# kezakool/flair-for-aigle

Hardware: AMD Instinct MI355X
Metric: 512x512x5 tiles/sec (train fwd+bwd+AdamW), U-Net ResNet-34, 19 classes (higher is better)
Workload: dtype bf16; 1 GPU; synthetic 512x512x5 tiles, 19-class U-Net (ResNet-34 encoder), batch 32 per GPU, train step (BASELINE.json configs[1]); global_batch=32, tile=512, parallelism=dp1

## Files before the change

### flair-for-aigle_amd/csrc/conv_pack.hip

```cpp
#include "ffa_common.h"

#include "conv7x7_stem.h"

struct PackDesc {
  const float* src;
  void* dst;
  const float* scale;
  long long s_row, s_ch;
  int rows, chs;
  int flip, kh, kw;
  int nchunks;
  int rg, bco, ncb;
  int ncb64;
  int mt, ci;
};


__device__ __forceinline__ void pack_eight(const PackDesc& p, long long i8, int dtype) {
  const int EPC = (dtype == FFA_BF16) ? 16 : 8;
  const int G8 = EPC / 8;
  const int taps = p.rg * p.kw;
  const int nrg = p.kh / p.rg;
  long long t = i8;
  const int e0 = (int)(t % G8) * 8; t /= G8;
  const int tap = t % taps; t /= taps;
  const int row_l = t % p.bco; t /= p.bco;
  const int rg = t % nrg; t /= nrg;
  const int cc = t % p.nchunks; t /= p.nchunks;
  const int cb = (int)t;
  int row_in_block = row_l;
  if (p.bco >= 64) {
    const int j = row_l & 63, mt = j >> 5, rho = j & 31;
    row_in_block = (row_l & ~63) + 16 * (rho >> 3) + 8 * ((rho >> 2) & 1) + 4 * mt + (rho & 3);
  }
  const int row = cb * p.bco + row_in_block;
  const int ch0 = cc * EPC + e0;
  int r = rg * p.rg + tap / p.kw;
  int sx = tap % p.kw;
  if (p.flip) {
    r = p.kh - 1 - r;
    sx = p.kw - 1 - sx;
  }
  float v[8];
  const bool row_ok = row < p.rows;
  const float sc = (row_ok && p.scale) ? p.scale[row] : 1.f;
  const float* src = p.src + (long long)row * p.s_row + r * p.kw + sx;
#pragma unroll
  for (int j = 0; j < 8; ++j) {
    const int ch = ch0 + j;
    v[j] = (row_ok && ch < p.chs) ? src[(long long)ch * p.s_ch] * sc : 0.f;
  }
  if (dtype == FFA_BF16)
    ffa_store8<ffa_bf16>(static_cast<ffa_bf16*>(p.dst) + i8 * 8, v);
  else
    ffa_store8<float>(static_cast<float*>(p.dst) + i8 * 8, v);
}

__global__ void pack_igemm_kernel(PackDesc one, const PackDesc* __restrict__ table, int dtype) {
  PackDesc p = one;
  if (table) p = table[blockIdx.y];
  const int EPC = (dtype == FFA_BF16) ? 16 : 8;
  const long long total8 = (long long)p.ncb * p.nchunks * (p.kh / p.rg) * p.bco * (p.rg * p.kw) * (EPC / 8);
  for (long long i = blockIdx.x * (long long)blockDim.x + threadIdx.x; i < total8;
       i += (long long)gridDim.x * blockDim.x)
    pack_eight(p, i, dtype);
}


template <typename T>
__device__ __forceinline__ void ring_pack_piece(const PackDesc& p, long long i16) {
  constexpr int EPF = ElemTraits<T>::kPerFrag;
  long long t = i16;
  const int hp = (int)(t % 2); t /= 2;
  const int row_l = (int)(t % 64); t /= 64;
  const int ks = (int)(t % 2); t /= 2;
  const int s = (int)(t % 3); t /= 3;
  const int r = (int)(t % 3); t /= 3;
  const int cc = (int)(t % p.nchunks); t /= p.nchunks;
  const int cb = (int)t;
  const int mt = row_l >> 5, rho = row_l & 31;
  const int row = cb * 64 + 16 * (rho >> 3) + 8 * ((rho >> 2) & 1) + 4 * mt + (rho & 3);
  const int hsrc = hp ^ ((row_l >> 3) & 1);
  const int ch0 = cc * (4 * EPF) + ks * (2 * EPF) + hsrc * EPF;
  int rr = r, ss = s;
  if (p.flip) {
    rr = 2 - r;
    ss = 2 - s;
  }
  float v[8];
  const bool row_ok = row < p.rows;
  const float sc = (row_ok && p.scale) ? p.scale[row] : 1.f;
  const float* src = p.src + (long long)row * p.s_row + rr * 3 + ss;
#pragma unroll
  for (int j = 0; j < EPF; ++j) {
    const int ch = ch0 + j;
    v[j] = (row_ok && ch < p.chs) ? src[(long long)ch * p.s_ch] * sc : 0.f;
  }
  if constexpr (EPF == 8) {
    ffa_store8<ffa_bf16>(static_cast<ffa_bf16*>(p.dst) + i16 * 8, v);
  } else {
    *reinterpret_cast<float4*>(static_cast<float*>(p.dst) + i16 * 4) = make_float4(v[0], v[1], v[2], v[3]);
  }
}

__device__ __forceinline__ void ring16_pack_rowslot(const PackDesc& p, long long idx) {
  long long t = idx;
  int row_l, sp, cc;
  if (!p.flip) {
    sp = (int)(t % 4); t /= 4;
    cc = (int)(t % p.nchunks); t /= p.nchunks;
    row_l = (int)(t % 64); t /= 64;
  } else {
    row_l = (int)(t % 64); t /= 64;
    sp = (int)(t % 4); t /= 4;
    cc = (int)(t % p.nchunks); t /= p.nchunks;
  }
  const int cb = (int)t;
  const int mt = row_l >> 4, kg = (row_l >> 2) & 3, i = row_l & 3;
  const int row = cb * 64 + 16 * kg + 4 * mt + i;
  const int slot = sp ^ (((row_l >> 2) & 1) << 1);
  const int ch0 = cc * 32 + slot * 8;
  const bool row_ok = row < p.rows;
  const float sc = (row_ok && p.scale) ? p.scale[row] : 1.f;
  float v[8][9];
  if (!p.flip && row_ok && ch0 + 8 <= p.chs && (p.s_row & 3) == 0 && ((size_t)p.src & 15) == 0) {
    const ffa_f32x4* src4 = reinterpret_cast<const ffa_f32x4*>(p.src + (long long)row * p.s_row + (long long)ch0 * 9);
    float f[72];
#pragma unroll
    for (int q = 0; q < 18; ++q) {
      const ffa_f32x4 t4 = src4[q];
      f[4 * q] = t4[0]; f[4 * q + 1] = t4[1]; f[4 * q + 2] = t4[2]; f[4 * q + 3] = t4[3];
    }
#pragma unroll
    for (int j = 0; j < 8; ++j)
#pragma unroll
      for (int tp = 0; tp < 9; ++tp) v[j][tp] = f[j * 9 + tp] * sc;
  } else {
#pragma unroll
    for (int j = 0; j < 8; ++j) {
      const int ch = ch0 + j;
      const bool ok = row_ok && ch < p.chs;
      const float* src = p.src + (long long)(ok ? row : 0) * p.s_row + (long long)(ok ? ch : 0) * p.s_ch;
#pragma unroll
      for (int tp = 0; tp < 9; ++tp) v[j][tp] = ok ? src[p.flip ? 8 - tp : tp] * sc : 0.f;
    }
  }
  ffa_bf16* dst = static_cast<ffa_bf16*>(p.dst) + ((((long long)cb * p.nchunks + cc) * 9) * 256 + row_l * 4 + sp) * 8;
#pragma unroll
  for (int tp = 0; tp < 9; ++tp) {
    float o[8];
#pragma unroll
    for (int j = 0; j < 8; ++j) o[j] = v[j][tp];
    ffa_store8<ffa_bf16>(dst + (long long)tp * 256 * 8, o);
  }
}

__global__ void pack_ring_kernel(PackDesc one, const PackDesc* __restrict__ table, int dtype) {
  PackDesc p = one;
  if (table) p = table[blockIdx.y];
  if (dtype == FFA_BF16) {
    const long long total = (long long)p.ncb64 * p.nchunks * 64 * 4;
    for (long long i = blockIdx.x * (long long)blockDim.x + threadIdx.x; i < total; i += (long long)gridDim.x * blockDim.x)
      ring16_pack_rowslot(p, i);
    return;
  }
  const long long total = (long long)p.ncb64 * p.nchunks * 3 * 3 * 2 * 64 * 2;
  for (long long i = blockIdx.x * (long long)blockDim.x + threadIdx.x; i < total; i += (long long)gridDim.x * blockDim.x)
    ring_pack_piece<float>(p, i);
}


__device__ __forceinline__ void thin_pack_piece(const PackDesc& p, int idx) {
  const int ks_n = (p.ci == 32) ? 9 : 5;
  const int lane = idx % 64;
  const int ks = (idx / 64) % ks_n;
  const int mt = idx / (64 * ks_n);
  const int r = lane & 15, kg = lane >> 4;
  const int q = r >> 2, i = r & 3;
  const int row = (p.mt == 2) ? (8 * q + 4 * mt + i) : (4 * q + i);
  int tap, ch0;
  if (p.ci == 32) {
    tap = ks;
    ch0 = 8 * kg;
  } else {
    tap = 2 * ks + (kg >> 1);
    ch0 = 8 * (kg & 1);
  }
  float v[8];
  const bool ok = row < p.rows && tap < 9;
  const float sc = (ok && p.scale) ? p.scale[row] : 1.f;
  const int st = p.flip ? 8 - tap : tap;
#pragma unroll
  for (int j = 0; j < 8; ++j) {
    const int ch = ch0 + j;
    v[j] = (ok && ch < p.chs) ? p.src[(long long)row * p.s_row + (long long)ch * p.s_ch + st] * sc : 0.f;
  }
  ffa_store8<ffa_bf16>(static_cast<ffa_bf16*>(p.dst) + (long long)idx * 8, v);
}

__global__ void pack_thin_kernel(PackDesc one, const PackDesc* __restrict__ table) {
  PackDesc p = one;
  if (table) p = table[blockIdx.y];
  const int total = p.mt * ((p.ci == 32) ? 9 : 5) * 64;
  for (int i = blockIdx.x * blockDim.x + threadIdx.x; i < total; i += gridDim.x * blockDim.x) thin_pack_piece(p, i);
}


__global__ void pack_stem_kernel(PackDesc one, const PackDesc* __restrict__ table) {
  PackDesc p = one;
  if (table) p = table[blockIdx.y];
  const int i = blockIdx.x * blockDim.x + threadIdx.x;
  if (i >= StemGeom::KSTEPS * 64 * 4) return;
  const int slotp = i & 3, rho = (i >> 2) & 63, ks = i >> 8;
  const int slot = slotp ^ (((rho >> 2) & 1) << 1);
  const int r = ks >> 1, s = 4 * (ks & 1) + slot;
  const int mt = rho >> 4, q = (rho >> 2) & 3, ii = rho & 3;
  const int co = 16 * q + 4 * mt + ii;
  unsigned short v[8];
#pragma unroll
  for (int c = 0; c < 8; ++c) {
    float x = 0.f;
    if (co < p.rows && c < p.chs && s < 7) {
      x = p.src[((size_t)(co * p.chs + c) * 7 + r) * 7 + s];
      if (p.scale) x *= p.scale[co];
    }
    v[c] = ffa_f32_to_bf16_bits(x);
  }
  uint4 u;
  u.x = v[0] | ((unsigned)v[1] << 16);
  u.y = v[2] | ((unsigned)v[3] << 16);
  u.z = v[4] | ((unsigned)v[5] << 16);
  u.w = v[6] | ((unsigned)v[7] << 16);
  reinterpret_cast<uint4*>(p.dst)[i] = u;
}


static int pack_fill(PackDesc& p, const float* w_oihw, const float* scale, void* dst, int O, int I_total, int col0,
                     int ncols, int kh, int kw, int transpose, int co_rows, int ci_pitch, int bco, int rg, int dtype) {
  FFA_REQUIRE(dtype == FFA_BF16 || dtype == FFA_F32, "pack: bad dtype");
  FFA_REQUIRE(w_oihw && dst, "pack: null pointer");
  FFA_REQUIRE(col0 >= 0 && ncols > 0 && col0 + ncols <= I_total, "pack: column block outside the tensor");
  const int eb = (dtype == FFA_BF16) ? 2 : 4;
  memset(&p, 0, sizeof(p));
  p.src = w_oihw + (long long)col0 * kh * kw;
  p.dst = dst;
  p.scale = scale;
  if (!transpose) {
    p.rows = O; p.chs = ncols;
    p.s_row = (long long)I_total * kh * kw;
    p.s_ch = (long long)kh * kw;
    p.flip = 0;
  } else {
    p.rows = ncols; p.chs = O;
    p.s_row = (long long)kh * kw;
    p.s_ch = (long long)I_total * kh * kw;
    p.flip = 1;
  }
  p.kh = kh; p.kw = kw;
  FFA_REQUIRE(p.rows <= co_rows && p.chs <= ci_pitch, "pack: padded dims smaller than the tensor");
  FFA_REQUIRE(ncols == I_total || !(bco & (FFA_BCO_STEM | FFA_BCO_THIN | FFA_BCO_RING)),
              "pack: a column block needs the conv_igemm layout");
  if (bco & FFA_BCO_STEM) {
    FFA_REQUIRE(kh == 7 && kw == 7 && dtype == FFA_BF16 && !transpose, "pack: the stem layout is for the bf16 7x7 forward operand");
    FFA_REQUIRE(O > 0 && O <= 64 && ncols > 0 && ncols <= 8, "stem pack: 1..64 output and 1..8 input channels, got %d / %d", O, ncols);
  } else if (bco & FFA_BCO_THIN) {
    FFA_REQUIRE(kh == 3 && kw == 3 && dtype == FFA_BF16, "pack: the thin layout is for bf16 3x3 kernels");
    FFA_REQUIRE((co_rows == 16 || co_rows == 32) && (ci_pitch == 16 || ci_pitch == 32), "thin pack: rows %d / pitch %d",
                co_rows, ci_pitch);
    p.mt = co_rows / 16;
    p.ci = ci_pitch;
  } else if (bco & FFA_BCO_RING) {
    FFA_REQUIRE(kh == 3 && kw == 3, "pack: the ring layout is for 3x3 kernels");
    FFA_REQUIRE(co_rows % 64 == 0 && (ci_pitch * eb) % 64 == 0, "ring pack: rows %d / pitch %d not whole groups", co_rows,
                ci_pitch);
    p.nchunks = ci_pitch * eb / 64;
    p.ncb64 = co_rows / 64;
  } else {
    FFA_REQUIRE(bco > 0 && co_rows % bco == 0, "pack: rows %d not a multiple of block %d", co_rows, bco);
    FFA_REQUIRE(rg > 0 && kh % rg == 0, "pack: bad row group");
    FFA_REQUIRE(ci_pitch % 16 == 0, "pack: channel pitch must be a multiple of 16");
    p.rg = rg; p.bco = bco;
    p.nchunks = ci_pitch * eb / 32;
    p.ncb = co_rows / bco;
  }
  return FFA_OK;
}

static int pack_launch(int dtype, int bco, const PackDesc& one, const PackDesc* table, int n, hipStream_t stream) {
  if (bco & FFA_BCO_STEM) {
    hipLaunchKernelGGL(pack_stem_kernel, dim3(ffa_cdiv(StemGeom::KSTEPS * 64 * 4, 256), n), dim3(256), 0, stream, one, table);
    return ffa_check_launch("pack_stem");
  }
  if (bco & FFA_BCO_THIN) {
    hipLaunchKernelGGL(pack_thin_kernel, dim3(5, n), dim3(256), 0, stream, one, table);
    return ffa_check_launch("pack_thin");
  }
  if (bco & FFA_BCO_RING) {
    hipLaunchKernelGGL(pack_ring_kernel, dim3(256, n), dim3(256), 0, stream, one, table, dtype);
    return ffa_check_launch("pack_ring");
  }
  hipLaunchKernelGGL(pack_igemm_kernel, dim3(256, n), dim3(256), 0, stream, one, table, dtype);
  return ffa_check_launch("pack_igemm");
}

extern "C" long long ffa_pack_conv_weight_bytes(int dtype, int co_rows, int ci_pitch, int kh, int kw, int bco) {
  if (bco & FFA_BCO_STEM) return StemGeom::WBYTES;
  if (bco & FFA_BCO_THIN) return (long long)(co_rows / 16) * ((ci_pitch == 32) ? 9 : 5) * 1024;
  const long long eb = (dtype == FFA_BF16) ? 2 : 4;
  return (long long)co_rows * ci_pitch * kh * kw * eb;
}

extern "C" int ffa_pack_conv_weight(int dtype, const float* w_oihw, const float* scale, void* dst, int O, int I,
                                    int kh, int kw, int transpose, int co_rows, int ci_pitch, int bco, int rg,
                                    hipStream_t stream) {
  PackDesc p;
  const int rc = pack_fill(p, w_oihw, scale, dst, O, I, 0, I, kh, kw, transpose, co_rows, ci_pitch, bco, rg, dtype);
  if (rc != FFA_OK) return rc;
  return pack_launch(dtype, bco, p, nullptr, 1, stream);
}

extern "C" int ffa_pack_desc_bytes(void) { return (int)sizeof(PackDesc); }

extern "C" int ffa_pack_desc_fill(void* host_desc, const float* w_oihw, const float* scale, void* dst, int O,
                                  int I_total, int col0, int ncols, int kh, int kw, int transpose, int co_rows,
                                  int ci_pitch, int bco, int rg, int dtype) {
  FFA_REQUIRE(host_desc, "pack_desc_fill: null pointer");
  PackDesc p;
  const int rc = pack_fill(p, w_oihw, scale, dst, O, I_total, col0, ncols, kh, kw, transpose, co_rows, ci_pitch, bco, rg,
                           dtype);
  if (rc != FFA_OK) return rc;
  memcpy(host_desc, &p, sizeof(p));
  return FFA_OK;
}

extern "C" int ffa_pack_conv_weights_batched(int dtype, int bco, const void* descs_device, int n, hipStream_t stream) {
  FFA_REQUIRE(dtype == FFA_BF16 || dtype == FFA_F32, "pack_batched: bad dtype");
  FFA_REQUIRE(descs_device && n > 0 && n <= 65535, "pack_batched: bad descriptor table");
  return pack_launch(dtype, bco, PackDesc{}, static_cast<const PackDesc*>(descs_device), n, stream);
}
```

### flair-for-aigle_amd/csrc/norm_pool.hip

```cpp
#include "ffa_common.h"

#define FFA_EW_THREADS 256
#define FFA_MAX_PARTIALS 1024
#ifndef FFA_EW_UNROLL
#define FFA_EW_UNROLL 4
#endif

static inline int ew_grid(long long items) {
  long long g = (items + FFA_EW_THREADS - 1) / FFA_EW_THREADS;
  if (g > 256 * 8) g = 256 * 8;
  if (g < 1) g = 1;
  return (int)g;
}

static inline int ew_grid_c(long long nvec, int C) {
  int a = C / 8, b = FFA_EW_THREADS;
  while (b) {
    const int r = a % b;
    a = b;
    b = r;
  }
  const int m = (C / 8) / a;
  const int g = ew_grid((nvec + FFA_EW_UNROLL - 1) / FFA_EW_UNROLL) / m * m;
  return g < m ? m : g;
// ... 709 lines not shown
  FFA_REQUIRE(relu != 1 || y, "bn_bwd: relu mode 1 needs the forward output");
  FFA_REQUIRE(C % 8 == 0 && C >= 8 && C <= 8 * FFA_EW_THREADS, "bn_bwd: unsupported channel count %d", C);
  if (workspace_bytes < ffa_bn_workspace_bytes(C)) {
    ffa_set_error("bn_bwd: workspace too small");
    return FFA_ERR_WORKSPACE;
  }
  const int nb = reduce_blocks(npix, C);
  float* ws = static_cast<float*>(workspace);
  const long long nvec = npix * (C / 8);
  const float inv_count = (float)(1.0 / (double)npix);
  float* coef = ws + (long long)FFA_MAX_PARTIALS * 2 * C;
  const bool g_in_dres = relu == 1 && dres != nullptr;
  if (g_in_dres) {
    const size_t bytes = (size_t)npix * C * (dtype == FFA_BF16 ? 2 : 4);
    const char* r = static_cast<const char*>(dres);
    auto overlaps = [&](const void* o) {
      const char* c = static_cast<const char*>(o);
      return c < r + bytes && r < c + bytes;
    };
    FFA_REQUIRE(!overlaps(x) && !overlaps(y) && !overlaps(dx), "bn_bwd: dres overlaps x, y or dx");
    FFA_REQUIRE(dres == dy || !overlaps(dy), "bn_bwd: dres may be dy itself, not a shifted view of it");
  }
  const void* ag = g_in_dres ? dres : dy;
  const void* ay = g_in_dres ? nullptr : y;
  void* ares = g_in_dres ? nullptr : dres;
  const int arelu = g_in_dres ? 0 : relu;
  if (dtype == FFA_BF16) {
    if ((stages & 5) && g_in_dres)
      hipLaunchKernelGGL((channel_reduce_kernel<ffa_bf16, BnBwdStoreOp>), dim3(nb), dim3(FFA_EW_THREADS), 0, stream,
                         (const ffa_bf16*)x, (const ffa_bf16*)dy, (const ffa_bf16*)y, mean, rstd, gamma, beta, ws, npix,
                         C, relu, (ffa_bf16*)dres);
    else if (stages & 5)
      hipLaunchKernelGGL((channel_reduce_kernel<ffa_bf16, BnBwdOp>), dim3(nb), dim3(FFA_EW_THREADS), 0, stream,
                         (const ffa_bf16*)x, (const ffa_bf16*)dy, (const ffa_bf16*)y, mean, rstd, gamma, beta, ws, npix,
                         C, relu, (ffa_bf16*)nullptr);
    if (stages & 9)
      hipLaunchKernelGGL(bn_bwd_finalize_kernel, dim3(ffa_cdiv(C, 8)), dim3(FFA_FIN_THREADS), 0, stream, ws, nb, C,
                         gamma, beta, mean, rstd, inv_count, dgamma, dbeta, coef);
    if (stages & 2)
      hipLaunchKernelGGL(bn_bwd_apply_kernel<ffa_bf16>, dim3(ew_grid_c(nvec, C)), dim3(FFA_EW_THREADS), 0, stream,
                         (const ffa_bf16*)x, (const ffa_bf16*)ag, (const ffa_bf16*)ay, coef, (ffa_bf16*)dx,
                         (ffa_bf16*)ares, nvec, C, arelu);
  } else {
    if ((stages & 5) && g_in_dres)
      hipLaunchKernelGGL((channel_reduce_kernel<float, BnBwdStoreOp>), dim3(nb), dim3(FFA_EW_THREADS), 0, stream,
                         (const float*)x, (const float*)dy, (const float*)y, mean, rstd, gamma, beta, ws, npix, C, relu,
                         (float*)dres);
    else if (stages & 5)
      hipLaunchKernelGGL((channel_reduce_kernel<float, BnBwdOp>), dim3(nb), dim3(FFA_EW_THREADS), 0, stream,
                         (const float*)x, (const float*)dy, (const float*)y, mean, rstd, gamma, beta, ws, npix, C, relu,
                         (float*)nullptr);
    if (stages & 9)
      hipLaunchKernelGGL(bn_bwd_finalize_kernel, dim3(ffa_cdiv(C, 8)), dim3(FFA_FIN_THREADS), 0, stream, ws, nb, C,
                         gamma, beta, mean, rstd, inv_count, dgamma, dbeta, coef);
    if (stages & 2)
      hipLaunchKernelGGL(bn_bwd_apply_kernel<float>, dim3(ew_grid_c(nvec, C)), dim3(FFA_EW_THREADS), 0, stream,
                         (const float*)x, (const float*)ag, (const float*)ay, coef, (float*)dx, (float*)ares, nvec, C,
                         arelu);
  }
  return ffa_check_launch("bn_bwd");
}


#define FFA_COOP_THREADS 512

__device__ __forceinline__ bool ffa_grid_barrier(unsigned* counter, unsigned nblocks, unsigned* fail) {
  __shared__ int ok_s;
  __syncthreads();
  if (threadIdx.x == 0) {
    __threadfence();
    atomicAdd(counter, 1u);
    int ok = 1;
    unsigned spins = 0;
    while (__hip_atomic_load(counter, __ATOMIC_ACQUIRE, __HIP_MEMORY_SCOPE_AGENT) < nblocks) {
      __builtin_amdgcn_s_sleep(16);
      if (++spins > (1u << 22)) {
        ok = 0;
        atomicExch(fail, 1u);
        break;
      }
    }
    __threadfence();
    ok_s = ok;
  }
  __syncthreads();
  return ok_s != 0;
}

__device__ __forceinline__ void ffa_unpack8_bf16(const ffa_u32x4& u, float (&v)[8]) {
  v[0] = __uint_as_float(u.x << 16); v[1] = __uint_as_float(u.x & 0xffff0000u);
  v[2] = __uint_as_float(u.y << 16); v[3] = __uint_as_float(u.y & 0xffff0000u);
  v[4] = __uint_as_float(u.z << 16); v[5] = __uint_as_float(u.z & 0xffff0000u);
  v[6] = __uint_as_float(u.w << 16); v[7] = __uint_as_float(u.w & 0xffff0000u);
}

template <int ITEMS>
__global__ void __launch_bounds__(FFA_COOP_THREADS, 1)
bn_bwd_coop_kernel(const ffa_bf16* __restrict__ x, const ffa_bf16* __restrict__ dy, const ffa_bf16* __restrict__ y,
                   const float* __restrict__ gamma, const float* __restrict__ beta, const float* __restrict__ mean,
                   const float* __restrict__ rstd, ffa_bf16* __restrict__ dx, ffa_bf16* __restrict__ dres,
                   float* __restrict__ dgamma, float* __restrict__ dbeta, float* __restrict__ ws,
                   unsigned* __restrict__ sync, long long nvec, int C, int relu, float inv_count) {
  __shared__ float red[FFA_COOP_THREADS][17];
  __shared__ double dred[FFA_COOP_THREADS / 64];
  const int CG = C / 8;
  const int t = threadIdx.x;
  const long long nthreads = (long long)gridDim.x * FFA_COOP_THREADS;
  const long long tid_g = (long long)blockIdx.x * FFA_COOP_THREADS + t;
  const int cg = (int)(tid_g % CG), c0 = cg * 8;
  float mu[8], rs[8], sc[8], sh[8];
#pragma unroll
  for (int e = 0; e < 8; ++e) {
    mu[e] = mean[c0 + e];
    rs[e] = rstd[c0 + e];
    sc[e] = (gamma ? gamma[c0 + e] : 1.f) * rs[e];
    sh[e] = (beta ? beta[c0 + e] : 0.f) - mu[e] * sc[e];
  }
  ffa_u32x4 xr[ITEMS], gr[ITEMS];
  float a[8], b[8];
#pragma unroll
  for (int e = 0; e < 8; ++e) a[e] = b[e] = 0.f;
#pragma unroll
  for (int k = 0; k < ITEMS; ++k) {
    const long long i = tid_g + (long long)k * nthreads;
    xr[k] = ffa_u32x4{0u, 0u, 0u, 0u};
    gr[k] = ffa_u32x4{0u, 0u, 0u, 0u};
    if (i < nvec) {
      xr[k] = *reinterpret_cast<const ffa_u32x4*>(x + i * 8);
      ffa_u32x4 g = *reinterpret_cast<const ffa_u32x4*>(dy + i * 8);
      float xv[8], gv[8];
      ffa_unpack8_bf16(xr[k], xv);
      unsigned keep = 0xffu;
      if (relu == 1) {
        float yv[8];
        ffa_unpack8_bf16(*reinterpret_cast<const ffa_u32x4*>(y + i * 8), yv);
        keep = 0;
#pragma unroll
        for (int e = 0; e < 8; ++e) keep |= (yv[e] > 0.f ? 1u : 0u) << e;
      } else if (relu == 2) {
        keep = 0;
#pragma unroll
        for (int e = 0; e < 8; ++e) keep |= ((xv[e] * sc[e] + sh[e]) > 0.f ? 1u : 0u) << e;
      }
      uint32_t w[4] = {g.x, g.y, g.z, g.w};
#pragma unroll
      for (int q = 0; q < 4; ++q)
        w[q] &= ((keep >> (2 * q)) & 1u ? 0x0000ffffu : 0u) | ((keep >> (2 * q + 1)) & 1u ? 0xffff0000u : 0u);
      gr[k] = ffa_u32x4{w[0], w[1], w[2], w[3]};
      ffa_unpack8_bf16(gr[k], gv);
#pragma unroll
      for (int e = 0; e < 8; ++e) {
        a[e] += gv[e];
        b[e] += gv[e] * (xv[e] - mu[e]) * rs[e];
      }
    }
  }
#pragma unroll
  for (int e = 0; e < 8; ++e) {
    red[t][e] = a[e];
    red[t][8 + e] = b[e];
  }
  __syncthreads();
  const int PL = FFA_COOP_THREADS / CG;
  for (int idx = t; idx < 2 * C; idx += FFA_COOP_THREADS) {
    const int which = idx / C, c = idx % C;
    const int g = c / 8, e = (c % 8) + which * 8;
    float s = 0.f;
    for (int q = 0; q < PL; ++q) s += red[q * CG + g][e];
    ws[((long long)blockIdx.x * 2 + which) * C + c] = s;
  }
  const unsigned nb = gridDim.x;
  bool ok = ffa_grid_barrier(sync + 0, nb, sync + 3);
  float* tot = ws + (long long)FFA_MAX_PARTIALS * 2 * C;
  for (int v = blockIdx.x; v < 2 * C; v += nb) {
    double s = 0.0;
    for (unsigned p = t; p < nb; p += FFA_COOP_THREADS) s += (double)ws[(long long)p * 2 * C + v];
#pragma unroll
    for (int o = 32; o > 0; o >>= 1) s += __shfl_xor(s, o, 64);
    if ((t & 63) == 0) dred[t >> 6] = s;
    __syncthreads();
    if (t == 0) {
      double r = 0.0;
      for (int wv = 0; wv < FFA_COOP_THREADS / 64; ++wv) r += dred[wv];
      tot[v] = (float)r;
    }
    __syncthreads();
  }
  ok = ffa_grid_barrier(sync + 1, nb, sync + 3) && ok;
  float kg[8], kx[8], k0[8];
#pragma unroll
  for (int e = 0; e < 8; ++e) {
    const float s = __hip_atomic_load(tot + c0 + e, __ATOMIC_RELAXED, __HIP_MEMORY_SCOPE_AGENT);
    const float q = __hip_atomic_load(tot + C + c0 + e, __ATOMIC_RELAXED, __HIP_MEMORY_SCOPE_AGENT);
    kg[e] = (gamma ? gamma[c0 + e] : 1.f) * rs[e];
    kx[e] = -kg[e] * rs[e] * q * inv_count;
    k0[e] = -kg[e] * s * inv_count - kx[e] * mu[e];
    if (blockIdx.x == 0 && t < CG) {
      dbeta[c0 + e] = s;
      dgamma[c0 + e] = q;
    }
  }
#pragma unroll
  for (int k = 0; k < ITEMS; ++k) {
    const long long i = tid_g + (long long)k * nthreads;
    if (i < nvec) {
      float xv[8], gv[8], o[8];
      ffa_unpack8_bf16(xr[k], xv);
      ffa_unpack8_bf16(gr[k], gv);
#pragma unroll
      for (int e = 0; e < 8; ++e) o[e] = kg[e] * gv[e] + kx[e] * xv[e] + k0[e];
      ffa_store8<ffa_bf16>(dx + i * 8, o);
      if (dres) *reinterpret_cast<ffa_u32x4*>(dres + i * 8) = gr[k];
    }
  }
  __syncthreads();
  if (t == 0) {
    __threadfence();
    if (atomicAdd(sync + 2, 1u) == nb - 1) {
      sync[0] = 0u;
      sync[1] = 0u;
      sync[2] = 0u;
      __threadfence();
    }
  }
  (void)ok;
}

extern "C" int ffa_bn_bwd_fused(int dtype, const void* x, const void* dy, const void* y, const float* gamma,
                                const float* beta, const float* mean, const float* rstd, void* dx, void* dres,
                                float* dgamma, float* dbeta, long long npix, int C, int relu, void* workspace,
                                long long workspace_bytes, unsigned* sync, hipStream_t stream) {
  FFA_REQUIRE(x && dy && dx && mean && rstd && dgamma && dbeta && workspace && sync, "bn_bwd_fused: null pointer");
  FFA_REQUIRE(relu >= 0 && relu <= 2 && (relu != 1 || y), "bn_bwd_fused: bad relu mode");
  static int cus = 0;
  if (cus == 0) {
    int dev = 0;
    hipDeviceProp_t prop;
    if (hipGetDevice(&dev) != hipSuccess || hipGetDeviceProperties(&prop, dev) != hipSuccess) return FFA_ERR_UNSUPPORTED;
    cus = prop.multiProcessorCount;
  }
  const int CG = C / 8;
  if (dtype != FFA_BF16 || C % 8 != 0 || CG < 1 || FFA_COOP_THREADS % CG != 0 || cus < 8 || cus > FFA_MAX_PARTIALS) {
    ffa_set_error("bn_bwd_fused: unsupported dtype / channel count %d", C);
    return FFA_ERR_UNSUPPORTED;
  }
  if (workspace_bytes < ffa_bn_workspace_bytes(C)) {
    ffa_set_error("bn_bwd_fused: workspace too small");
    return FFA_ERR_WORKSPACE;
  }
  const long long nvec = npix * CG;
  const long long nthreads = (long long)cus * FFA_COOP_THREADS;
  const long long items = (nvec + nthreads - 1) / nthreads;
  if (items > 16) {
    ffa_set_error("bn_bwd_fused: %lld vectors per thread exceed the register budget", items);
    return FFA_ERR_UNSUPPORTED;
  }
  const float inv_count = (float)(1.0 / (double)npix);
#define FFA_COOP_LAUNCH(N_)                                                                                      \
  hipLaunchKernelGGL(bn_bwd_coop_kernel<N_>, dim3(cus), dim3(FFA_COOP_THREADS), 0, stream, (const ffa_bf16*)x,   \
                     (const ffa_bf16*)dy, (const ffa_bf16*)y, gamma, beta, mean, rstd, (ffa_bf16*)dx,            \
                     (ffa_bf16*)dres, dgamma, dbeta, (float*)workspace, sync, nvec, C, relu, inv_count)
  if (items <= 4) FFA_COOP_LAUNCH(4);
  else FFA_COOP_LAUNCH(16);
#undef FFA_COOP_LAUNCH
  return ffa_check_launch("bn_bwd_fused");
}

extern "C" int ffa_bn_bwd_partials(int dtype, const void* x, const void* dy, const float* partials, long long nparts,
                                   const float* gamma, const float* beta, const float* mean, const float* rstd,
                                   void* dx, float* dgamma, float* dbeta, long long npix, int C, void* workspace,
                                   long long workspace_bytes, hipStream_t stream) {
  FFA_REQUIRE(x && dy && partials && dx && mean && rstd && dgamma && dbeta && workspace, "bn_bwd_partials: null pointer");
  FFA_REQUIRE(C % 8 == 0 && C >= 8 && C <= 8 * FFA_EW_THREADS && nparts > 0, "bn_bwd_partials: bad arguments");
  if (workspace_bytes < ffa_bn_workspace_bytes(C)) {
    ffa_set_error("bn_bwd_partials: workspace too small");
    return FFA_ERR_WORKSPACE;
  }
  float* ws = static_cast<float*>(workspace);
  float* coef = ws + (long long)FFA_MAX_PARTIALS * 2 * C;
  const float* src = partials;
  int n = (int)nparts;
  if (nparts > FFA_MAX_PARTIALS) {
    const int R = 64;
    hipLaunchKernelGGL(partials_fold_kernel, dim3(ffa_cdiv(C, 8), R), dim3(FFA_FIN_THREADS), 0, stream, partials, nparts,
                       C, R, ws);
    src = ws;
    n = R;
  }
  const long long nvec = npix * (C / 8);
  const float inv_count = (float)(1.0 / (double)npix);
  hipLaunchKernelGGL(bn_bwd_finalize_kernel, dim3(ffa_cdiv(C, 8)), dim3(FFA_FIN_THREADS), 0, stream, src, n, C, gamma, beta,
                     mean, rstd, inv_count, dgamma, dbeta, coef, 1);
  if (dtype == FFA_BF16)
    hipLaunchKernelGGL(bn_bwd_apply_kernel<ffa_bf16>, dim3(ew_grid_c(nvec, C)), dim3(FFA_EW_THREADS), 0, stream,
                       (const ffa_bf16*)x, (const ffa_bf16*)dy, (const ffa_bf16*)nullptr, coef, (ffa_bf16*)dx,
                       (ffa_bf16*)nullptr, nvec, C, 2);
  else
    hipLaunchKernelGGL(bn_bwd_apply_kernel<float>, dim3(ew_grid_c(nvec, C)), dim3(FFA_EW_THREADS), 0, stream, (const float*)x,
                       (const float*)dy, (const float*)nullptr, coef, (float*)dx, (float*)nullptr, nvec, C, 2);
  return ffa_check_launch("bn_bwd_partials");
}


template <typename T>
__global__ void __launch_bounds__(FFA_EW_THREADS)
maxpool_fwd_kernel(const T* __restrict__ x, T* __restrict__ y, uint8_t* __restrict__ idx, int B, int H, int W, int C,
                   int Ho, int Wo) {
  const unsigned CG = C / 8;
  const int oy = blockIdx.x % Ho;
  const long long b = blockIdx.x / Ho;
  const long long row = (long long)blockIdx.x * Wo * CG;
  for (unsigned j = threadIdx.x; j < (unsigned)Wo * CG; j += FFA_EW_THREADS) {
    const int ox = (int)(j / CG), g = (int)(j % CG);
    const long long i = row + j;
    float best[8];
    int bi[8];
#pragma unroll
    for (int e = 0; e < 8; ++e) {
      best[e] = -INFINITY;
      bi[e] = 0;
    }
    bool first = true;
#pragma unroll
    for (int r = 0; r < 3; ++r) {
      const int iy = oy * 2 - 1 + r;
      if (iy < 0 || iy >= H) continue;
#pragma unroll
      for (int s = 0; s < 3; ++s) {
        const int ix = ox * 2 - 1 + s;
        if (ix < 0 || ix >= W) continue;
        float v[8];
        ffa_load8<T>(x + ((b * H + iy) * W + ix) * C + g * 8, v);
#pragma unroll
        for (int e = 0; e < 8; ++e) {
          if (first || v[e] > best[e] || v[e] != v[e]) {
            best[e] = v[e];
            bi[e] = r * 3 + s;
          }
        }
        first = false;
      }
    }
    ffa_store8<T>(y + i * 8, best);
    uint32_t lo = bi[0] | (bi[1] << 8) | (bi[2] << 16) | (bi[3] << 24);
    uint32_t hi = bi[4] | (bi[5] << 8) | (bi[6] << 16) | (bi[7] << 24);
    *reinterpret_cast<uint2*>(idx + i * 8) = make_uint2(lo, hi);
  }
}

template <typename T>
__global__ void __launch_bounds__(FFA_EW_THREADS)
maxpool_bwd_kernel(const T* __restrict__ dy, const uint8_t* __restrict__ idx, const T* __restrict__ add,
                   T* __restrict__ dx, int B, int H, int W, int C, int Ho, int Wo) {
  const unsigned CG = C / 8;
  const int iy = blockIdx.x % H;
  const long long b = blockIdx.x / H;
  const long long row = (long long)blockIdx.x * W * CG;
  for (unsigned j = threadIdx.x; j < (unsigned)W * CG; j += FFA_EW_THREADS) {
    const int ix = (int)(j / CG), g = (int)(j % CG);
    const long long i = row + j;
    const int ny = (iy & 1) ? 2 : 1, nx = (ix & 1) ? 2 : 1;
    const int oy_c[2] = {(iy & 1) ? (iy + 1) >> 1 : iy >> 1, (iy - 1) >> 1};
    const int r_c[2] = {(iy & 1) ? 0 : 1, 2};
    const int ox_c[2] = {(ix & 1) ? (ix + 1) >> 1 : ix >> 1, (ix - 1) >> 1};
    const int s_c[2] = {(ix & 1) ? 0 : 1, 2};
    float acc[8];
#pragma unroll
    for (int e = 0; e < 8; ++e) acc[e] = 0.f;
    Raw8<T> addr, gr[4];
    uint2 kk[4];
    bool ok[4];
    if (add) addr.load(add + i * 8);
#pragma unroll
    for (int c = 0; c < 4; ++c) {
      const int cy = c >> 1, cx = c & 1;
      ok[c] = cy < ny && cx < nx && oy_c[cy] >= 0 && oy_c[cy] < Ho && ox_c[cx] >= 0 && ox_c[cx] < Wo;
      const long long o = ok[c] ? (((b * Ho + oy_c[cy]) * Wo + ox_c[cx]) * CG + g) * 8 : 0;
      kk[c] = *reinterpret_cast<const uint2*>(idx + o);
      gr[c].load(dy + o);
    }
    if (add) addr.get(acc);
#pragma unroll
    for (int c = 0; c < 4; ++c) {
      if (!ok[c]) continue;
      const int tap = r_c[c >> 1] * 3 + s_c[c & 1];
      float gv[8];
      gr[c].get(gv);
#pragma unroll
      for (int e = 0; e < 8; ++e) {
        const uint32_t word = e < 4 ? kk[c].x : kk[c].y;
        const int wq = (word >> (8 * (e & 3))) & 0xff;
        if (wq == tap) acc[e] += gv[e];
      }
    }
    ffa_store8<T>(dx + i * 8, acc);
  }
}

extern "C" int ffa_maxpool3x3s2_fwd(int dtype, const void* x, void* y, uint8_t* idx, int B, int H, int W, int C,
                                    hipStream_t stream) {
  FFA_REQUIRE(x && y && idx && C % 8 == 0, "maxpool_fwd: bad arguments");
  const int Ho = (H + 2 - 3) / 2 + 1, Wo = (W + 2 - 3) / 2 + 1;
  FFA_REQUIRE(B > 0 && (long long)B * Ho < (1LL << 31), "maxpool_fwd: too many rows");
  const int rows = B * Ho;
  if (dtype == FFA_BF16)
    hipLaunchKernelGGL(maxpool_fwd_kernel<ffa_bf16>, dim3(rows), dim3(FFA_EW_THREADS), 0, stream,
                       (const ffa_bf16*)x, (ffa_bf16*)y, idx, B, H, W, C, Ho, Wo);
  else
    hipLaunchKernelGGL(maxpool_fwd_kernel<float>, dim3(rows), dim3(FFA_EW_THREADS), 0, stream,
                       (const float*)x, (float*)y, idx, B, H, W, C, Ho, Wo);
  return ffa_check_launch("maxpool_fwd");
}

extern "C" int ffa_maxpool3x3s2_bwd(int dtype, const void* dy, const uint8_t* idx, const void* add, void* dx, int B,
                                    int H, int W, int C, hipStream_t stream) {
  FFA_REQUIRE(dy && dx && idx && C % 8 == 0, "maxpool_bwd: bad arguments");
  const int Ho = (H + 2 - 3) / 2 + 1, Wo = (W + 2 - 3) / 2 + 1;
  FFA_REQUIRE(B > 0 && (long long)B * H < (1LL << 31), "maxpool_bwd: too many rows");
  const int rows = B * H;
  if (dtype == FFA_BF16)
    hipLaunchKernelGGL(maxpool_bwd_kernel<ffa_bf16>, dim3(rows), dim3(FFA_EW_THREADS), 0, stream,
                       (const ffa_bf16*)dy, idx, (const ffa_bf16*)add, (ffa_bf16*)dx, B, H, W, C, Ho, Wo);
  else
    hipLaunchKernelGGL(maxpool_bwd_kernel<float>, dim3(rows), dim3(FFA_EW_THREADS), 0, stream,
                       (const float*)dy, idx, (const float*)add, (float*)dx, B, H, W, C, Ho, Wo);
  return ffa_check_launch("maxpool_bwd");
}

extern "C" int ffa_channel_sums(int dtype, const void* x, long long npix, int C, float* sum_out, float* sumsq_out,
                                void* workspace, long long workspace_bytes, hipStream_t stream) {
  FFA_REQUIRE(x && sum_out && sumsq_out && workspace, "channel_sums: null pointer");
  FFA_REQUIRE(C % 8 == 0 && C >= 8 && C <= 8 * FFA_EW_THREADS, "channel_sums: unsupported channel count %d", C);
  if (workspace_bytes < ffa_bn_workspace_bytes(C)) {
    ffa_set_error("channel_sums: workspace too small");
    return FFA_ERR_WORKSPACE;
  }
  const int nb = reduce_blocks(npix, C);
  float* ws = static_cast<float*>(workspace);
  if (dtype == FFA_BF16)
    hipLaunchKernelGGL((channel_reduce_kernel<ffa_bf16, StatOp>), dim3(nb), dim3(FFA_EW_THREADS), 0, stream,
                       (const ffa_bf16*)x, (const ffa_bf16*)nullptr, (const ffa_bf16*)nullptr, nullptr, nullptr, nullptr, nullptr, ws,
                       npix, C, 0, (ffa_bf16*)nullptr);
  else
    hipLaunchKernelGGL((channel_reduce_kernel<float, StatOp>), dim3(nb), dim3(FFA_EW_THREADS), 0, stream,
                       (const float*)x, (const float*)nullptr, (const float*)nullptr, nullptr, nullptr, nullptr, nullptr, ws, npix,
                       C, 0, (float*)nullptr);
  hipLaunchKernelGGL(bn_bwd_finalize_kernel, dim3(ffa_cdiv(C, 8)), dim3(FFA_FIN_THREADS), 0, stream, ws, nb, C,
                     (const float*)nullptr, (const float*)nullptr, (const float*)nullptr, (const float*)nullptr, 0.f,
                     sumsq_out, sum_out, (float*)nullptr);
  return ffa_check_launch("channel_sums");
}
```

Measured before the change: 2411 tiles/s.

## Stage ring weight pack through LDS and reuse input rows in maxpool kernels

Adds a bf16 ring-pack path for flipped 3x3 weights. It loads contiguous fp32 runs with vector loads into a shared-memory stage, then writes the transposed packed layout from there, replacing strided per-element gathers. The maxpool forward now computes two output rows per block from five shared input rows, so overlapping window rows are loaded once. The maxpool backward makes each thread handle a 2x2 input patch, which reuses the loaded dy and index values. Grids shrink accordingly, and register pressure and LDS use go up.

```diff
diff --git a/flair-for-aigle_amd/csrc/conv_pack.hip b/flair-for-aigle_amd/csrc/conv_pack.hip
--- a/flair-for-aigle_amd/csrc/conv_pack.hip
+++ b/flair-for-aigle_amd/csrc/conv_pack.hip
@@ -155,10 +155,88 @@
   }
 }
 
+#define RING16_RUN (64 * 9)
+__device__ __forceinline__ void ring16_pack_unit_transposed(const PackDesc& p, int unit,
+                                                            unsigned short (*__restrict__ stage)[RING16_RUN]) {
+  const int tid = threadIdx.x;
+  const int cc = unit % p.nchunks, cb = unit / p.nchunks;
+  const int nrow = p.rows - cb * 64 < 64 ? p.rows - cb * 64 : 64;
+  const int nval = nrow > 0 ? nrow * 9 : 0;
+  constexpr int V4 = RING16_RUN / 4;
+#pragma unroll 1
+  for (int h = 0; h < 18; h += 9) {
+  ffa_f32x4 f[9];
+#pragma unroll
+  for (int k = 0; k < 9; ++k) {
+    const int q = tid + 256 * (h + k);
+    const int chl = q / V4, e4 = (q % V4) * 4;
+    const int ch = cc * 32 + chl;
+    f[k] = ffa_f32x4{0.f, 0.f, 0.f, 0.f};
+    if (ch < p.chs && e4 < nval) {
+      const float* src = p.src + (long long)ch * p.s_ch + (long long)cb * RING16_RUN + e4;
+      if (e4 + 4 <= nval) {
+        f[k] = *reinterpret_cast<const ffa_f32x4*>(src);
+      } else {
+#pragma unroll
+        for (int u = 0; u < 4; ++u)
+          if (e4 + u < nval) f[k][u] = src[u];
+      }
+    }
+  }
+#pragma unroll
+  for (int k = 0; k < 9; ++k) {
+    const int q = tid + 256 * (h + k);
+    const int chl = q / V4, e4 = (q % V4) * 4;
+    unsigned short b[4];
+    if (p.scale) {
+      const int r0 = e4 / 9, left = 9 * (r0 + 1) - e4;
+      const bool ch_ok = cc * 32 + chl < p.chs;
+      const bool ok0 = ch_ok && e4 < nval, ok1 = ch_ok && e4 + left < nval;
+      const float sc0 = ok0 ? p.scale[cb * 64 + r0] : 1.f, sc1 = ok1 ? p.scale[cb * 64 + r0 + 1] : 1.f;
+#pragma unroll
+      for (int u = 0; u < 4; ++u) {
+        const bool ok = u < left ? ok0 : ok1;
+        b[u] = ffa_f32_to_bf16_bits(ok ? f[k][u] * (u < left ? sc0 : sc1) : 0.f);
+      }
+    } else {
+#pragma unroll
+      for (int u = 0; u < 4; ++u) b[u] = ffa_f32_to_bf16_bits(f[k][u]);
+    }
+    *reinterpret_cast<uint2*>(&stage[chl][e4]) =
+        make_uint2(b[0] | ((unsigned)b[1] << 16), b[2] | ((unsigned)b[3] << 16));
+  }
+  }
+  __syncthreads();
+  const int row_l = tid & 63, sp = tid >> 6;
+  const int mt = row_l >> 4, kg = (row_l >> 2) & 3, i = row_l & 3;
+  const int rin = 16 * kg + 4 * mt + i;
+  const int slot = sp ^ (((row_l >> 2) & 1) << 1);
+  ffa_bf16* dst = static_cast<ffa_bf16*>(p.dst) + ((((long long)cb * p.nchunks + cc) * 9) * 256 + row_l * 4 + sp) * 8;
+#pragma unroll
+  for (int tp = 0; tp < 9; ++tp) {
+    unsigned short b[8];
+#pragma unroll
+    for (int j = 0; j < 8; ++j) b[j] = stage[slot * 8 + j][rin * 9 + 8 - tp];
+    uint4 u;
+    u.x = b[0] | ((unsigned)b[1] << 16);
+    u.y = b[2] | ((unsigned)b[3] << 16);
+    u.z = b[4] | ((unsigned)b[5] << 16);
+    u.w = b[6] | ((unsigned)b[7] << 16);
+    *reinterpret_cast<uint4*>(dst + (long long)tp * 256 * 8) = u;
+  }
+  __syncthreads();
+}
+
 __global__ void pack_ring_kernel(PackDesc one, const PackDesc* __restrict__ table, int dtype) {
   PackDesc p = one;
   if (table) p = table[blockIdx.y];
   if (dtype == FFA_BF16) {
+    if (p.flip && p.s_row == 9 && (p.s_ch & 3) == 0 && ((size_t)p.src & 15) == 0) {
+      __shared__ __align__(16) unsigned short stage[32][RING16_RUN];
+      const int units = p.ncb64 * p.nchunks;
+      for (int unit = blockIdx.x; unit < units; unit += gridDim.x) ring16_pack_unit_transposed(p, unit, stage);
+      return;
+    }
     const long long total = (long long)p.ncb64 * p.nchunks * 64 * 4;
     for (long long i = blockIdx.x * (long long)blockDim.x + threadIdx.x; i < total; i += (long long)gridDim.x * blockDim.x)
       ring16_pack_rowslot(p, i);
diff --git a/flair-for-aigle_amd/csrc/norm_pool.hip b/flair-for-aigle_amd/csrc/norm_pool.hip
--- a/flair-for-aigle_amd/csrc/norm_pool.hip
+++ b/flair-for-aigle_amd/csrc/norm_pool.hip
@@ -1035,49 +1035,80 @@
 }
 
 
+
+template <typename T, int R0>
+__device__ __forceinline__ void maxpool_window(const Raw8<T> (&v)[5][3], const bool (&rok)[5], const bool (&cok)[3],
+                                               T* __restrict__ y, uint8_t* __restrict__ idx) {
+  float best[8];
+  int bi[8];
+#pragma unroll
+  for (int e = 0; e < 8; ++e) {
+    best[e] = -INFINITY;
+    bi[e] = 0;
+  }
+  bool first = true;
+#pragma unroll
+  for (int r = 0; r < 3; ++r) {
+#pragma unroll
+    for (int s = 0; s < 3; ++s) {
+      if (!(rok[R0 + r] && cok[s])) continue;
+      float f[8];
+      v[R0 + r][s].get(f);
+#pragma unroll
+      for (int e = 0; e < 8; ++e) {
+        if (first || f[e] > best[e] || f[e] != f[e]) {
+          best[e] = f[e];
+          bi[e] = r * 3 + s;
+        }
+      }
+      first = false;
+    }
+  }
+  ffa_store8<T>(y, best);
+  uint32_t lo = bi[0] | (bi[1] << 8) | (bi[2] << 16) | (bi[3] << 24);
+  uint32_t hi = bi[4] | (bi[5] << 8) | (bi[6] << 16) | (bi[7] << 24);
+  *reinterpret_cast<uint2*>(idx) = make_uint2(lo, hi);
+}
+
 template <typename T>
 __global__ void __launch_bounds__(FFA_EW_THREADS)
 maxpool_fwd_kernel(const T* __restrict__ x, T* __restrict__ y, uint8_t* __restrict__ idx, int B, int H, int W, int C,
                    int Ho, int Wo) {
   const unsigned CG = C / 8;
-  const int oy = blockIdx.x % Ho;
-  const long long b = blockIdx.x / Ho;
-  const long long row = (long long)blockIdx.x * Wo * CG;
+  const int Hb = (Ho + 1) / 2;
+  const int oy = (int)(blockIdx.x % Hb) * 2;
+  const long long b = blockIdx.x / Hb;
+  const bool two = oy + 1 < Ho;
+  bool rok[5];
+  long long rbase[5];
+#pragma unroll
+  for (int r = 0; r < 5; ++r) {
+    const int iy = oy * 2 - 1 + r;
+    rok[r] = iy >= 0 && iy < H;
+    rbase[r] = (b * H + (rok[r] ? iy : oy * 2)) * W;
+  }
+  const long long row = (b * Ho + oy) * Wo * CG;
   for (unsigned j = threadIdx.x; j < (unsigned)Wo * CG; j += FFA_EW_THREADS) {
     const int ox = (int)(j / CG), g = (int)(j % CG);
+    bool cok[3];
+    int col[3];
+#pragma unroll
+    for (int s = 0; s < 3; ++s) {
+      const int ix = ox * 2 - 1 + s;
+      cok[s] = ix >= 0 && ix < W;
+      col[s] = cok[s] ? ix : ox * 2;
+    }
+    Raw8<T> v[5][3];
+#pragma unroll
+    for (int r = 0; r < 5; ++r)
+#pragma unroll
+      for (int s = 0; s < 3; ++s) v[r][s].load(x + (rbase[r] + col[s]) * C + g * 8);
     const long long i = row + j;
-    float best[8];
-    int bi[8];
-#pragma unroll
-    for (int e = 0; e < 8; ++e) {
-      best[e] = -INFINITY;
-      bi[e] = 0;
-    }
-    bool first = true;
-#pragma unroll
-    for (int r = 0; r < 3; ++r) {
-      const int iy = oy * 2 - 1 + r;
-      if (iy < 0 || iy >= H) continue;
-#pragma unroll
-      for (int s = 0; s < 3; ++s) {
-        const int ix = ox * 2 - 1 + s;
-        if (ix < 0 || ix >= W) continue;
-        float v[8];
-        ffa_load8<T>(x + ((b * H + iy) * W + ix) * C + g * 8, v);
-#pragma unroll
-        for (int e = 0; e < 8; ++e) {
-          if (first || v[e] > best[e] || v[e] != v[e]) {
-            best[e] = v[e];
-            bi[e] = r * 3 + s;
-          }
-        }
-        first = false;
-      }
-    }
-    ffa_store8<T>(y + i * 8, best);
-    uint32_t lo = bi[0] | (bi[1] << 8) | (bi[2] << 16) | (bi[3] << 24);
-    uint32_t hi = bi[4] | (bi[5] << 8) | (bi[6] << 16) | (bi[7] << 24);
-    *reinterpret_cast<uint2*>(idx + i * 8) = make_uint2(lo, hi);
+    maxpool_window<T, 0>(v, rok, cok, y + i * 8, idx + i * 8);
+    if (two) {
+      const long long i2 = i + (long long)Wo * CG;
+      maxpool_window<T, 2>(v, rok, cok, y + i2 * 8, idx + i2 * 8);
+    }
   }
 }
 
@@ -1086,47 +1117,55 @@
 maxpool_bwd_kernel(const T* __restrict__ dy, const uint8_t* __restrict__ idx, const T* __restrict__ add,
                    T* __restrict__ dx, int B, int H, int W, int C, int Ho, int Wo) {
   const unsigned CG = C / 8;
-  const int iy = blockIdx.x % H;
-  const long long b = blockIdx.x / H;
-  const long long row = (long long)blockIdx.x * W * CG;
-  for (unsigned j = threadIdx.x; j < (unsigned)W * CG; j += FFA_EW_THREADS) {
-    const int ix = (int)(j / CG), g = (int)(j % CG);
-    const long long i = row + j;
-    const int ny = (iy & 1) ? 2 : 1, nx = (ix & 1) ? 2 : 1;
-    const int oy_c[2] = {(iy & 1) ? (iy + 1) >> 1 : iy >> 1, (iy - 1) >> 1};
-    const int r_c[2] = {(iy & 1) ? 0 : 1, 2};
-    const int ox_c[2] = {(ix & 1) ? (ix + 1) >> 1 : ix >> 1, (ix - 1) >> 1};
-    const int s_c[2] = {(ix & 1) ? 0 : 1, 2};
-    float acc[8];
-#pragma unroll
-    for (int e = 0; e < 8; ++e) acc[e] = 0.f;
-    Raw8<T> addr, gr[4];
+  const int Hb = (H + 1) / 2, Wb = (W + 1) / 2;
+  const int m = (int)(blockIdx.x % Hb);
+  const long long b = blockIdx.x / Hb;
+  for (unsigned j = threadIdx.x; j < (unsigned)Wb * CG; j += FFA_EW_THREADS) {
+    const int n = (int)(j / CG), g = (int)(j % CG);
+    bool ook[4], pok[4];
+    long long po[4];
+    Raw8<T> addr[4], gr[4];
     uint2 kk[4];
-    bool ok[4];
-    if (add) addr.load(add + i * 8);
-#pragma unroll
-    for (int c = 0; c < 4; ++c) {
-      const int cy = c >> 1, cx = c & 1;
-      ok[c] = cy < ny && cx < nx && oy_c[cy] >= 0 && oy_c[cy] < Ho && ox_c[cx] >= 0 && ox_c[cx] < Wo;
-      const long long o = ok[c] ? (((b * Ho + oy_c[cy]) * Wo + ox_c[cx]) * CG + g) * 8 : 0;
-      kk[c] = *reinterpret_cast<const uint2*>(idx + o);
-      gr[c].load(dy + o);
-    }
-    if (add) addr.get(acc);
-#pragma unroll
-    for (int c = 0; c < 4; ++c) {
-      if (!ok[c]) continue;
-      const int tap = r_c[c >> 1] * 3 + s_c[c & 1];
-      float gv[8];
-      gr[c].get(gv);
-#pragma unroll
-      for (int e = 0; e < 8; ++e) {
-        const uint32_t word = e < 4 ? kk[c].x : kk[c].y;
-        const int wq = (word >> (8 * (e & 3))) & 0xff;
-        if (wq == tap) acc[e] += gv[e];
-      }
-    }
-    ffa_store8<T>(dx + i * 8, acc);
+#pragma unroll
+    for (int q = 0; q < 4; ++q) {
+      const int cy = q >> 1, cx = q & 1;
+      ook[q] = m + cy < Ho && n + cx < Wo;
+      const long long o = (((b * Ho + (ook[q] ? m + cy : m)) * Wo + (ook[q] ? n + cx : n)) * CG + g) * 8;
+      kk[q] = *reinterpret_cast<const uint2*>(idx + o);
+      gr[q].load(dy + o);
+      pok[q] = 2 * m + cy < H && 2 * n + cx < W;
+      po[q] = (((b * H + (pok[q] ? 2 * m + cy : 2 * m)) * W + (pok[q] ? 2 * n + cx : 2 * n)) * CG + g) * 8;
+      if (add) addr[q].load(add + po[q]);
+    }
+#pragma unroll
+    for (int q = 0; q < 4; ++q) {
+      if (!pok[q]) continue;
+      const int py = q >> 1, px = q & 1;
+      float acc[8];
+#pragma unroll
+      for (int e = 0; e < 8; ++e) acc[e] = 0.f;
+      if (add) addr[q].get(acc);
+#pragma unroll
+      for (int u = 0; u < (py ? 2 : 1); ++u) {
+        const int cy = py ? 1 - u : 0, r = py ? 2 * u : 1;
+#pragma unroll
+        for (int w = 0; w < (px ? 2 : 1); ++w) {
+          const int cx = px ? 1 - w : 0, s = px ? 2 * w : 1;
+          const int oq = cy * 2 + cx;
+          if (!ook[oq]) continue;
+          const int tap = r * 3 + s;
+          float gv[8];
+          gr[oq].get(gv);
+#pragma unroll
+          for (int e = 0; e < 8; ++e) {
+            const uint32_t word = e < 4 ? kk[oq].x : kk[oq].y;
+            const int wq = (word >> (8 * (e & 3))) & 0xff;
+            if (wq == tap) acc[e] += gv[e];
+          }
+        }
+      }
+      ffa_store8<T>(dx + po[q], acc);
+    }
   }
 }
 
@@ -1135,12 +1174,12 @@
   FFA_REQUIRE(x && y && idx && C % 8 == 0, "maxpool_fwd: bad arguments");
   const int Ho = (H + 2 - 3) / 2 + 1, Wo = (W + 2 - 3) / 2 + 1;
   FFA_REQUIRE(B > 0 && (long long)B * Ho < (1LL << 31), "maxpool_fwd: too many rows");
-  const int rows = B * Ho;
+  const int blocks = B * ((Ho + 1) / 2);
   if (dtype == FFA_BF16)
-    hipLaunchKernelGGL(maxpool_fwd_kernel<ffa_bf16>, dim3(rows), dim3(FFA_EW_THREADS), 0, stream,
+    hipLaunchKernelGGL(maxpool_fwd_kernel<ffa_bf16>, dim3(blocks), dim3(FFA_EW_THREADS), 0, stream,
                        (const ffa_bf16*)x, (ffa_bf16*)y, idx, B, H, W, C, Ho, Wo);
   else
-    hipLaunchKernelGGL(maxpool_fwd_kernel<float>, dim3(rows), dim3(FFA_EW_THREADS), 0, stream,
+    hipLaunchKernelGGL(maxpool_fwd_kernel<float>, dim3(blocks), dim3(FFA_EW_THREADS), 0, stream,
                        (const float*)x, (float*)y, idx, B, H, W, C, Ho, Wo);
   return ffa_check_launch("maxpool_fwd");
 }
@@ -1150,12 +1189,12 @@
   FFA_REQUIRE(dy && dx && idx && C % 8 == 0, "maxpool_bwd: bad arguments");
   const int Ho = (H + 2 - 3) / 2 + 1, Wo = (W + 2 - 3) / 2 + 1;
   FFA_REQUIRE(B > 0 && (long long)B * H < (1LL << 31), "maxpool_bwd: too many rows");
-  const int rows = B * H;
+  const int blocks = B * ((H + 1) / 2);
   if (dtype == FFA_BF16)
-    hipLaunchKernelGGL(maxpool_bwd_kernel<ffa_bf16>, dim3(rows), dim3(FFA_EW_THREADS), 0, stream,
+    hipLaunchKernelGGL(maxpool_bwd_kernel<ffa_bf16>, dim3(blocks), dim3(FFA_EW_THREADS), 0, stream,
                        (const ffa_bf16*)dy, idx, (const ffa_bf16*)add, (ffa_bf16*)dx, B, H, W, C, Ho, Wo);
   else
-    hipLaunchKernelGGL(maxpool_bwd_kernel<float>, dim3(rows), dim3(FFA_EW_THREADS), 0, stream,
+    hipLaunchKernelGGL(maxpool_bwd_kernel<float>, dim3(blocks), dim3(FFA_EW_THREADS), 0, stream,
                        (const float*)dy, idx, (const float*)add, (float*)dx, B, H, W, C, Ho, Wo);
   return ffa_check_launch("maxpool_bwd");
 }
```

Measured after the change: 2420 tiles/s (median of 6 runs). About the same (+0.4%).
